# ligengen/EgoGen

Hardware: AMD Instinct MI355X
Metric: PPO env-steps/sec (512 parallel SMPL-X agents) (higher is better)
Workload: dtype f32 (blend GEMM: shape/template columns as 2-term bf16 splits, pose correctives as one fp16 product, fp32 accumulate); PPO update products on 2-term bf16 splits; rollout policy layers on 2-term bf16 splits

## Files before the change

egogen_amd/_lib.py:

```python
from __future__ import annotations

import ctypes as C
import os

_HERE = os.path.dirname(os.path.abspath(__file__))
LIB_PATH = os.path.join(_HERE, "libegogen_hip.so")

c_float_p = C.POINTER(C.c_float)
c_int_p = C.POINTER(C.c_int32)


class EgxError(RuntimeError):
    pass


class BodyModelHost(C.Structure):
    _fields_ = [
        ("num_verts", C.c_int),
        ("v_template_host", C.c_void_p), ("shapedirs_host", C.c_void_p), ("posedirs_host", C.c_void_p),
        ("J_regressor_host", C.c_void_p), ("parents_host", C.c_void_p), ("lbs_weights_host", C.c_void_p),
        ("hand_comps_l_host", C.c_void_p), ("hand_comps_r_host", C.c_void_p),
        ("hand_mean_l_host", C.c_void_p), ("hand_mean_r_host", C.c_void_p),
        ("extra_vids_host", C.c_void_p), ("lmk_vids_host", C.c_void_p), ("lmk_bary_host", C.c_void_p),
        ("num_markers", C.c_int), ("marker_vids_host", C.c_void_p),
# ... 227 lines not shown
    "egx_policy_train_create": (C.c_int, [C.POINTER(PolicyWeights), C.POINTER(PolicyGrads), C.c_int, C.POINTER(C.c_void_p)]),
    "egx_policy_train_destroy": (None, [C.c_void_p]),
    "egx_policy_train_refresh": (C.c_int, [C.c_void_p, C.c_void_p]),
    "egx_policy_train_packed": (C.c_int, [C.c_void_p, C.POINTER(PolicyPacked3)]),
    "egx_policy_train_bind": (C.c_int, [C.c_void_p, C.c_void_p, C.c_void_p]),
    "egx_policy_train_step": (C.c_int, [C.c_void_p] * 9 + [C.c_float] * 6 + [C.c_void_p, C.c_void_p]),
    "egx_policy_train_step_heads": (C.c_int, [C.c_void_p] * 9 + [C.c_float] * 6 + [C.c_void_p, C.c_void_p]),
    "egx_policy_train_step_encoders": (C.c_int, [C.c_void_p, C.c_void_p]),
    "egx_policy_train_set_precision": (C.c_int, [C.c_void_p, C.c_int]),
    "egx_policy_train_dense3_launches": (C.c_int, [C.c_void_p]),
    "egx_policy_train_head": (C.c_int, [C.c_void_p, C.POINTER(UpdateHead), C.c_void_p]),
    "egx_policy_train_step_cursor": (C.c_int, [C.c_void_p, C.POINTER(UpdateHead), C.c_void_p] + [C.c_float] * 6 + [C.c_void_p]),
    "egx_policy_train_step_heads_cursor": (C.c_int, [C.c_void_p, C.POINTER(UpdateHead), C.c_void_p] + [C.c_float] * 6 + [C.c_void_p]),
    "egx_adamw_clip_step_cursor": (C.c_int, [C.c_void_p, C.c_void_p, C.c_void_p, C.c_void_p, C.c_size_t, C.c_size_t, C.c_float] +
                                   [C.c_double] * 5 + [C.c_void_p, C.c_void_p, C.c_void_p, C.c_void_p]),
    "egx_pack3_bytes": (C.c_size_t, [C.c_int, C.c_int]),
    "egx_pack3": (C.c_int, [C.c_void_p, C.c_int, C.c_int, C.c_int, C.c_int, C.c_void_p, C.c_int, C.c_int, C.c_void_p]),
    "egx_gemm3_workspace_bytes": (C.c_size_t, [C.c_int, C.c_int, C.c_int]),
    "egx_gemm3": (C.c_int, [C.c_void_p, C.c_int, C.c_int, C.c_void_p, C.c_int, C.c_int, C.c_int, C.c_int, C.c_int, C.c_void_p, C.c_int,
                            C.c_float, C.c_void_p, C.c_int, C.c_void_p, C.c_int, C.c_void_p, C.c_int, C.c_void_p, C.c_size_t, C.c_void_p]),
    "egx_vposer_workspace_bytes": (C.c_size_t, [C.c_int]),
    "egx_vposer_encode": (C.c_int, [C.POINTER(VposerWeights), C.c_void_p, C.c_int, C.c_int, C.c_void_p, C.c_void_p,
                                    C.c_size_t, C.c_void_p]),
}

_lib = None


def load():
    global _lib
# ... 38 lines not shown
```

egogen_amd/csrc/egx_nets.h:

```cpp
#pragma once
#include "egx_common.h"
#include "egx_frame.h"

struct EgxSeg {
  const float* p;
  int w, ld;
};

int egx_launch_linear(hipStream_t st, int M, int N, const EgxSeg* segs, int nseg, const float* W, const float* b,
                      int act, float slope, const float* res, int ldr, float* out, int ldo);
int egx_launch_gru_pointwise(hipStream_t st, const float* gi, const float* gh, const float* hprev, int ldh, float* hout,
                             int ldo, int M, int H);
int egx_launch_cont6d_to_aa(hipStream_t st, const float* xb6, int n, float* out, int ldo);
int egx_launch_posenc(hipStream_t st, const float* dist, const float* time, int A, float* out);

void egx_launch_frame_scan(hipStream_t st, float* y, const float* x_last, int x_ld, int A, int width, int T);

struct D3Pack {
  const float* src;
  int R, K, ld, col0;
  void* dst;
  int S_total, s0;
  int transpose = 0;
};
// ... 26 lines not shown
  int S3T = 0, s3T0 = 0;
  float* bias_out = nullptr;
  int n_split = 0;
};
constexpr int EGX_DENSE3_MAX = 12;
int egx_launch_dense3_n(hipStream_t st, const D3Plain* ps, int n);
enum { EGX_DENSE3_BASE = 0, EGX_DENSE3_DEEP = 1, EGX_DENSE3_WIDE = 2 };
int egx_dense3_config(const D3Plain* ps, int n);
void egx_launch_dense3(hipStream_t st, const D3Plain& p);
void egx_launch_dense3_pair(hipStream_t st, const D3Plain& p, const D3Plain& q);
void egx_launch_dense3_triple(hipStream_t st, const D3Plain& p, const D3Plain& q, const D3Plain& r);
int egx_ppo_loss_packed_precleared(const float* zp, const float* value, const float* act, const float* adv, const float* ret,
                                   const float* logp_old, const float* adv_stats, const float* scale, float adv_eps, float min_logvar,
                                   float max_logvar, float eps_clip, float vf_coef, float ent_coef, int num_rows, float* g_zp,
                                   float* g_value, float* out_terms, void* stream_, const int* cursor = nullptr, int max_cursor = 0);
void egx_launch_posenc3(hipStream_t st, const float* dist, const float* time, int n, float* out, int ld, void* out3, int S3, int s0,
                        void* out3T = nullptr, int S3T = 0, int col0T = 0, float* zero6 = nullptr );

#if defined(__HIPCC__)
struct EgxRowsIdentity {
  __device__ __forceinline__ size_t operator()(int r) const { return (size_t)r; }
};
struct EgxRowsGathered {
  const long long* __restrict__ idx;
  int num_src;
  __device__ __forceinline__ size_t operator()(int r) const {
    const long long s = idx[r];
    return (size_t)min(max(s, 0LL), (long long)num_src - 1);
  }
};
// ... 97 lines not shown
```

egogen_amd/csrc/ppo.hip:

```cpp
#include <algorithm>
#include <cstring>
#include "egx_nets.h"

namespace {
constexpr float LOG_SQRT_2PI = 0.91893853320467274178f;

}

__device__ __forceinline__ float egx_wave_sum(float v) {
#pragma unroll
  for (int o = 32; o > 0; o >>= 1) v += __shfl_xor(v, o);
  return v;
}

__global__ __launch_bounds__(256) void egx_ppo_loss_kernel(const float* __restrict__ mu, const float* __restrict__ logvar,
                                                          const float* __restrict__ value, const float* __restrict__ act,
                                                          const float* __restrict__ adv, const float* __restrict__ ret,
                                                          const float* __restrict__ logp_old, const float* __restrict__ adv_stats,
                                                          const float* __restrict__ scale_ptr, float adv_eps, float min_lv,
                                                          float max_lv, float eps_clip, float vf_coef, float ent_coef, int n,
                                                          int stride ,
                                                          float* __restrict__ g_mu, float* __restrict__ g_logvar,
                                                          float* __restrict__ g_value, float* __restrict__ out_terms,
                                                          const int* __restrict__ cursor, int max_cursor) {
// ... 252 lines not shown
    const double t = (double)*step;
    const float bc1 = (float)(1.0 - pow(b1, t)), bc2 = (float)(1.0 - pow(b2, t));
    float coef = 1.f;
    if (do_clip) coef = fminf(max_norm / ((float)sqrt(red[0]) + 1e-6f), 1.f);
    consts[0] = coef;
    consts[1] = (float)(lr / bc1);
    consts[2] = sqrtf(bc2);
    if (cursor) *cursor += 1;
  }
}

__global__ __launch_bounds__(256) void egx_adamw_flat_kernel(float* __restrict__ p, const float* __restrict__ g, float* __restrict__ m,
                                                             float* __restrict__ v, size_t n, size_t n_clip,
                                                             const float* __restrict__ consts ,
                                                             double lr, double b1, double b2, double eps, double wd) {
  const float coef = consts[0], step_size = consts[1], bc2s = consts[2];
  const size_t i0 = ((size_t)blockIdx.x * 256 + threadIdx.x) * 4;
  if (i0 >= n) return;
  const int cnt = (int)((n - i0 < 4) ? (n - i0) : 4);
  float gr[4], pv[4], mv[4], vv[4];
  if (cnt == 4) {
    *reinterpret_cast<float4*>(gr) = *reinterpret_cast<const float4*>(g + i0);
    *reinterpret_cast<float4*>(pv) = *reinterpret_cast<const float4*>(p + i0);
    *reinterpret_cast<float4*>(mv) = *reinterpret_cast<const float4*>(m + i0);
    *reinterpret_cast<float4*>(vv) = *reinterpret_cast<const float4*>(v + i0);
  } else {
    for (int e = 0; e < cnt; ++e) { gr[e] = g[i0 + e]; pv[e] = p[i0 + e]; mv[e] = m[i0 + e]; vv[e] = v[i0 + e]; }
  }
  const double omb1 = 1.0 - b1, omb2 = 1.0 - b2, lrwd = lr * wd;
#pragma unroll
  for (int e = 0; e < 4; ++e) {
    if (e < cnt) {
      float gg = gr[e];
      if (i0 + e < n_clip) gg *= coef;
      pv[e] = (float)((double)pv[e] - lrwd * (double)pv[e]);
      mv[e] = (float)((double)mv[e] + omb1 * ((double)gg - (double)mv[e]));
      vv[e] = (float)(b2 * (double)vv[e] + omb2 * (double)gg * (double)gg);
      const float denom = (float)((double)(sqrtf(vv[e]) / bc2s) + eps);
      pv[e] -= step_size * mv[e] / denom;
    }
  }
  if (cnt == 4) {
    *reinterpret_cast<float4*>(p + i0) = *reinterpret_cast<const float4*>(pv);
    *reinterpret_cast<float4*>(m + i0) = *reinterpret_cast<const float4*>(mv);
    *reinterpret_cast<float4*>(v + i0) = *reinterpret_cast<const float4*>(vv);
  } else {
    for (int e = 0; e < cnt; ++e) { p[i0 + e] = pv[e]; m[i0 + e] = mv[e]; v[i0 + e] = vv[e]; }
  }
}

__global__ void egx_zero_terms_kernel(float* __restrict__ t) {
  if (threadIdx.x < 6) t[threadIdx.x] = 0.f;
}

static int ppo_loss_blocks(int num_rows) { return std::max(1, std::min(256, egx_ceil_div(num_rows, 8))); }

// ... 112 lines not shown
extern "C" int egx_rollout_store(const float* state, const float* egosensing, const float* dist, const float* time, const float* rew,
                                 const int32_t* term, int num_agents, float* state_dst, float* ego_dst, float* dist_dst, float* time_dst,
                                 float* rew_dst, int32_t* term_dst, float* ep_ret, float* ep_len, float* done_sums, void* stream_) {
  EGX_REQUIRE(state && egosensing && dist && time && state_dst && ego_dst && dist_dst && time_dst && num_agents > 0, "bad arguments");
  EGX_REQUIRE((!rew_dst && !term_dst && !ep_ret) || (rew && term && rew_dst && term_dst), "reward / termination source or slot missing");
  EGX_REQUIRE(!ep_ret || (ep_len && done_sums && rew && term), "episode bookkeeping needs ep_len, done_sums, rew, term");
  hipLaunchKernelGGL(egx_rollout_store_kernel, dim3(num_agents + (ep_ret ? 1 : 0)), dim3(256), 0, static_cast<hipStream_t>(stream_), state,
                     egosensing, dist, time, rew, term, num_agents, state_dst, ego_dst, dist_dst, time_dst, rew_dst, term_dst, ep_ret, ep_len,
                     done_sums);
  EGX_HIP_CHECK(hipGetLastError());
  return EGX_OK;
}

extern "C" size_t egx_adamw_workspace_floats(void) { return 1024 + 8; }

static int adamw_clip_step(float* param, const float* grad, float* exp_avg, float* exp_avg_sq, size_t n, size_t n_clip,
                           float max_norm, double lr, double beta1, double beta2, double eps, double weight_decay,
                           float* step, float* workspace, int* cursor, void* stream_) {
  EGX_REQUIRE(param && grad && exp_avg && exp_avg_sq && step && workspace && n > 0 && n_clip <= n, "bad arguments");
  hipStream_t st = static_cast<hipStream_t>(stream_);
  const int nb = 1024;
  const bool do_clip = max_norm > 0.f && n_clip > 0;
  hipLaunchKernelGGL(egx_sumsq_partial_kernel, dim3(nb), dim3(256), 0, st, grad, do_clip ? n_clip : (size_t)0, workspace, step);
  hipLaunchKernelGGL(egx_adamw_consts_kernel, dim3(1), dim3(256), 0, st, workspace, nb, do_clip ? 1 : 0, max_norm, lr, beta1, beta2,
                     step, workspace + nb, cursor);
  const size_t blocks = (n + 1023) / 1024;
  hipLaunchKernelGGL(egx_adamw_flat_kernel, dim3((unsigned)blocks), dim3(256), 0, st, param, grad, exp_avg, exp_avg_sq, n, n_clip,
                     workspace + nb, lr, beta1, beta2, eps, weight_decay);
  EGX_HIP_CHECK(hipGetLastError());
  return EGX_OK;
}

extern "C" int egx_adamw_clip_step(float* param, const float* grad, float* exp_avg, float* exp_avg_sq, size_t n, size_t n_clip,
                                   float max_norm, double lr, double beta1, double beta2, double eps, double weight_decay,
                                   float* step, float* workspace, void* stream_) {
  return adamw_clip_step(param, grad, exp_avg, exp_avg_sq, n, n_clip, max_norm, lr, beta1, beta2, eps, weight_decay, step, workspace,
                         nullptr, stream_);
}

extern "C" int egx_adamw_clip_step_cursor(float* param, const float* grad, float* exp_avg, float* exp_avg_sq, size_t n, size_t n_clip,
                                          float max_norm, double lr, double beta1, double beta2, double eps, double weight_decay,
                                          float* step, float* workspace, int32_t* cursor, void* stream_) {
  return adamw_clip_step(param, grad, exp_avg, exp_avg_sq, n, n_clip, max_norm, lr, beta1, beta2, eps, weight_decay, step, workspace,
                         cursor, stream_);
}
```

egogen_amd/csrc/update3.hip:

```cpp
#include <algorithm>
#include <cstdlib>
#include <cstring>
#include <vector>
#include "d3.h"

namespace {

struct PackEntry {
  const float* src;
  int red, cols, ld, col0;
  bf16x8* dst;
  int S_total, s0;
  int transpose;
  int ones_row;
  int frag_end;
  bf16x8* dst2;
  int S_total2;
};

template <class Rows>
__device__ __forceinline__ void u3_pack_fragment(const PackEntry& e, const float* __restrict__ src, int frag, int lane, int nplanes,
                                                 const Rows& rows) {
  float x[8];
  int rt, s;
// ... 67 lines not shown
    __builtin_amdgcn_wave_barrier();
#pragma unroll
    for (int t = 0; t < 2; ++t) {
#pragma unroll
      for (int q = 0; q < 8; ++q) x[q] = sb[8 * kg + q][16 * t + r];
      bf16x8 pl[3];
      d3_split(x, pl);
      bf16x8* o = e.dst2 + ((size_t)(2 * bj + t) * e.S_total2 + bi) * 3 * 64 + lane;
#pragma unroll
      for (int p = 0; p < 3; ++p)
        if (p < nplanes) o[p * 64] = pl[p];
    }
    return;
  }
  u3_pack_fragment(e, e.src, frag, lane, nplanes, EgxRowsIdentity());
}

struct HeadArgs {
  const PackEntry* tab;
  int n_tab, frags_tab, nplanes;
  const float *state, *ego;
  const long long* perm;
  const int* cursor;
  int max_cursor, n, num_src;
  const float *dist, *time, *act, *adv, *ret, *logp;
  float *act_c, *adv_c, *ret_c, *logp_c;
  float* stats;
  float* log;
  float* pe_out;
  int pe_ld;
// ... 171 lines not shown
struct egx_policy_train {
  int n = 0, Sn = 0;
  Arena ar;
  Encoder enc[2];
  Branch br[2];
  float* catf = nullptr;
  bf16x8 *cat_r = nullptr, *catT = nullptr;
  PackEntry* tab_weights = nullptr; int n_weights = 0, frags_weights = 0;
  PackEntry* tab_inputs = nullptr; int n_inputs = 0, frags_inputs = 0;
  PackEntry* tab_loss = nullptr; int n_loss = 0, frags_loss = 0;
  std::vector<PackEntry> h_inputs;
  const float* bound_state = nullptr; const float* bound_ego = nullptr;
  int prec = 0;
  int dense3_launches = 0;
  bool merge = true;
};

namespace {

int upload_table(std::vector<PackEntry>& v, PackEntry** dev, int* frags) {
  int run = 0;
  for (PackEntry& e : v) {
    if (e.transpose == 2) {
      run += egx_ceil_div(e.red, 32) * egx_ceil_div(e.cols, 32);
    } else {
      const int rows = e.transpose ? e.cols + (e.ones_row >= 0 ? 1 : 0) : e.red;
      const int red = e.transpose ? e.red : e.cols;
      run += (int)d3_img_frags(rows, red);
    }
    e.frag_end = run;
// ... 42 lines not shown
  const int lane = (row & 15) + 16 * kg;
  bf16x8 one;
#pragma unroll
  for (int e = 0; e < 8; ++e) one[e] = (short)0x3F80;
  img[((size_t)(row >> 4) * S_total + s) * 3 * 64 + lane] = one;
}

}

extern "C" int egx_policy_train_create(const egx_policy_weights* w, const egx_policy_grads* g, int num_rows, egx_policy_train** out) {
  EGX_REQUIRE(w && g && out, "null argument");
  EGX_REQUIRE(num_rows > 0 && num_rows % 32 == 0, "the minibatch must be a multiple of 32 rows");
  auto* h = new egx_policy_train();
  h->n = num_rows; h->Sn = num_rows / 32;
  if (const char* e = getenv("EGX_UPDATE_MERGE")) h->merge = !(e[0] == '0' && e[1] == 0);
  Encoder& X = h->enc[0];
  X.Wih = w->x_enc_w_ih; X.Whh = w->x_enc_w_hh; X.bih = w->x_enc_b_ih; X.bhh = w->x_enc_b_hh;
  X.gWih = g->x_enc_w_ih; X.gWhh = g->x_enc_w_hh; X.gbih = g->x_enc_b_ih; X.gbhh = g->x_enc_b_hh;
  X.in_dim = ST_DIM; X.cat_off = 0;
  Encoder& E = h->enc[1];
  E.Wih = w->ego_enc_w_ih; E.Whh = w->ego_enc_w_hh; E.bih = w->ego_enc_b_ih; E.bhh = w->ego_enc_b_hh;
  E.gWih = g->ego_enc_w_ih; E.gWhh = g->ego_enc_w_hh; E.gbih = g->ego_enc_b_ih; E.gbhh = g->ego_enc_b_hh;
  E.in_dim = EGO_DIM; E.cat_off = HD;
  for (int l = 0; l < 4; ++l) {
    h->br[0].W[l] = w->actor_w[l]; h->br[0].b[l] = w->actor_b[l]; h->br[0].gW[l] = g->actor_w[l]; h->br[0].gb[l] = g->actor_b[l];
    h->br[1].W[l] = w->critic_w[l]; h->br[1].b[l] = w->critic_b[l]; h->br[1].gW[l] = g->critic_w[l]; h->br[1].gb[l] = g->critic_b[l];
  }
  h->br[0].Wout = w->actor_out_w; h->br[0].bout = w->actor_out_b; h->br[0].gWout = g->actor_out_w; h->br[0].gbout = g->actor_out_b;
  h->br[0].nout = ZP;
  h->br[1].Wout = w->critic_out_w; h->br[1].bout = w->critic_out_b; h->br[1].gWout = g->critic_out_w; h->br[1].gbout = g->critic_out_b;
// ... 35 lines not shown
  for (int e = 0; e < 2; ++e) {
    Encoder& En = h->enc[e];
    add(tw, En.Wih, 3 * HD, En.in_dim, En.in_dim, 0, En.Wih_r, egx_ceil_div(En.in_dim, 32), 0, 0, -1);
    add_both(tw, En.Whh, 3 * HD, HD, En.Whh_r, En.Whh_t);
  }
  for (int b = 0; b < 2; ++b) {
    Branch& B = h->br[b];
    for (int l = 0; l < 4; ++l) {
      add_both(tw, B.W[l], CAT, CAT, B.W_r[l], B.W_t[l]);
    }
    add_both(tw, B.Wout, B.nout, CAT, B.Wout_r, B.Wout_t);
  }
  h->n_weights = (int)tw.size();
  int rc = upload_table(tw, &h->tab_weights, &h->frags_weights);
  if (rc) return fail(rc);
  for (int e = 0; e < 2; ++e) {
    Encoder& En = h->enc[e];
    const int d = En.in_dim, S = egx_ceil_div(d, 32);
    add(h->h_inputs, nullptr, n, d, 2 * d, 0, En.x0_r, S, 0, 0, -1);
    add(h->h_inputs, nullptr, n, d, 2 * d, d, En.x1_r, S, 0, 0, -1);
    add(h->h_inputs, nullptr, n, d, 2 * d, 0, En.xT, 2 * Sn, 0, 1, d);
    add(h->h_inputs, nullptr, n, d, 2 * d, d, En.xT, 2 * Sn, Sn, 1, d);
  }
  h->n_inputs = (int)h->h_inputs.size();
  if ((rc = upload_table(h->h_inputs, &h->tab_inputs, &h->frags_inputs))) return fail(rc);
  std::vector<PackEntry> tl;
  for (int b = 0; b < 2; ++b) {
    Branch& B = h->br[b];
    add(tl, B.ghead, n, B.nout, B.nout, 0, B.ghead_r, egx_ceil_div(B.nout, 32), 0, 0, -1);
    add(tl, B.ghead, n, B.nout, B.nout, 0, B.gheadT, Sn, 0, 1, -1);
  }
  h->n_loss = (int)tl.size();
  if ((rc = upload_table(tl, &h->tab_loss, &h->frags_loss))) return fail(rc);
  U3_CHECK(hipDeviceSynchronize());
#undef U3_CHECK
  *out = h;
  return EGX_OK;
}

extern "C" void egx_policy_train_destroy(egx_policy_train* h) {
  if (!h) return;
  (void)hipFree(h->ar.base); (void)hipFree(h->tab_weights); (void)hipFree(h->tab_inputs); (void)hipFree(h->tab_loss);
  delete h;
}

extern "C" int egx_policy_train_refresh(egx_policy_train* h, void* stream) {
  EGX_REQUIRE(h, "null handle");
  const int planes = std::max(d3_planes(h->prec), d3_planes(egx_policy_get_precision()));
  run_table(static_cast<hipStream_t>(stream), h->tab_weights, h->n_weights, h->frags_weights, planes);
  EGX_HIP_CHECK(hipGetLastError());
  return EGX_OK;
}

extern "C" int egx_policy_train_set_precision(egx_policy_train* h, int prec) {
  EGX_REQUIRE(h, "null handle");
  EGX_REQUIRE(prec == 0 || prec == 1 || prec == 2, "precision must be 0 (three bf16 planes: fp32-equivalent), 2 (two planes) or 1 (bf16)");
  h->prec = prec;
  return EGX_OK;
}

extern "C" int egx_policy_train_dense3_launches(const egx_policy_train* h) { return h ? h->dense3_launches : -1; }

extern "C" int egx_policy_train_packed(const egx_policy_train* h, egx_policy_packed3* out) {
  EGX_REQUIRE(h && out, "null argument");
  out->x_enc_w_ih = h->enc[0].Wih_r; out->x_enc_w_hh = h->enc[0].Whh_r;
  out->ego_enc_w_ih = h->enc[1].Wih_r; out->ego_enc_w_hh = h->enc[1].Whh_r;
// ... 304 lines not shown
```

egogen_amd/ppo_policy.py:

```python
from __future__ import annotations

import contextlib
import ctypes as C
import math
import os
import warnings
from typing import Dict, List, Optional

import numpy as np
import torch
import torch.distributed as dist
from torch import nn

from . import _lib
from .models import ActorCritic, GAMMAActor, GAMMACritic, GAMMAPolicyBase, PolicyHipRunner

_EPS = float(np.finfo(np.float32).eps)
_LOG_SQRT_2PI = math.log(math.sqrt(2 * math.pi))
_UPDATE_PREC = {"f32": 0, "bf16x2": 2, "bf16": 1}
_LOSS_ROWS, _OBS_ROWS = ("act", "adv", "ret", "logp_old"), ("state", "egosensing", "dist", "time")


class RunningMeanStd:

# ... 269 lines not shown
        g = _lib.PolicyGrads()
        s, a, c = self.shared_net, self.actor.pnet, self.critic.vnet
        gp = lambda t: t.grad.data_ptr()
        g.x_enc_w_ih, g.x_enc_w_hh, g.x_enc_b_ih, g.x_enc_b_hh = gp(s.x_enc.weight_ih_l0), gp(s.x_enc.weight_hh_l0), gp(s.x_enc.bias_ih_l0), gp(s.x_enc.bias_hh_l0)
        g.ego_enc_w_ih, g.ego_enc_w_hh, g.ego_enc_b_ih, g.ego_enc_b_hh = (gp(s.ego_enc.weight_ih_l0), gp(s.ego_enc.weight_hh_l0),
                                                                            gp(s.ego_enc.bias_ih_l0), gp(s.ego_enc.bias_hh_l0))
        for b in range(2):
            for k in range(2):
                g.actor_w[2 * b + k], g.actor_b[2 * b + k] = gp(a.layers[b].layers[k].weight), gp(a.layers[b].layers[k].bias)
                g.critic_w[2 * b + k], g.critic_b[2 * b + k] = gp(c.layers[b].layers[k].weight), gp(c.layers[b].layers[k].bias)
        g.actor_out_w, g.actor_out_b = gp(a.out_fc.weight), gp(a.out_fc.bias)
        g.critic_out_w, g.critic_out_b = gp(c.out_fc.weight), gp(c.out_fc.bias)
        h = C.c_void_p()
        _lib.check(lib.egx_policy_train_create(C.byref(w), C.byref(g), int(n), C.byref(h)), "egx_policy_train_create")
        _lib.check(lib.egx_policy_train_set_precision(h, _UPDATE_PREC[self.update_precision]), "egx_policy_train_set_precision")
        f = dict(dtype=torch.float32, device=self._flat_grad.device)
        head = os.environ.get("EGX_UPDATE_HEAD", "1") != "0"
        obs = [] if head else [torch.empty(n, k, **f) for k in (804, 64, 1, 1)]
        loss = [torch.empty(n, k, **f) for k in (128, 1, 1, 1)]
        if not head:
            _lib.check(lib.egx_policy_train_bind(h, _lib.ptr(obs[0]), _lib.ptr(obs[1])), "egx_policy_train_bind")
        packed = _lib.PolicyPacked3()
        _lib.check(lib.egx_policy_train_packed(h, C.byref(packed)), "egx_policy_train_packed")
        hs = {"h": h, "n": int(n), "head": head, "packed": packed, "stats": torch.zeros(2, **f),
              **dict(zip(_LOSS_ROWS, loss)), **dict(zip(_OBS_ROWS, obs))}
        self._train_handles[n] = hs
        if len(self._train_handles) == 1:
            self._runner.adopt_packed(packed, refresh=self._refresh_images)
        self._refresh_images()
        return hs

    def _chain_shapes_ok(self) -> bool:
        ok = getattr(self, "_chain_ok", None)
        if ok is None:
            a, c, s = self.actor.pnet, self.critic.vnet, self.shared_net
            def block_ok(blk, nout):
                return (blk.residual and len(blk.layers) == 2 and blk.out_fc.out_features == nout and blk.out_fc.in_features == 1152
                        and all(m.act_name == "lrelu" and len(m.layers) == 2 and
                                all(fc.in_features == 1152 and fc.out_features == 1152 for fc in m.layers) for m in blk.layers))
# ... 8 lines not shown
        self._train_handles = {}
        self._runner._wstruct = None

    def __del__(self):
        try:
            self._drop_train_handles()
        except Exception:
            pass

    def _prec_key(self):
        return (int(_lib.load().egx_policy_get_precision()), self.update_precision)

    def _img_key_now(self):
        return (sum(int(p._version) for p in self.parameters()), self._prec_key())

    def _refresh_images(self):
        if not self._train_handles:
            return
        lib, st = _lib.load(), _lib.current_stream_ptr()
        for hs in self._train_handles.values():
            _lib.check(lib.egx_policy_train_refresh(hs["h"], st), "egx_policy_train_refresh")
        self._img_key = self._img_key_now()
        self.refresh_counts["total"] += 1

    def _refresh_images_if_stale(self, who: str):
        if self._train_handles and self._img_key != self._img_key_now():
            self._refresh_images()
            self.refresh_counts[who] += 1

    def _fwd_bwd_train_step(self, hs, batch, idx, gstats, log_out, part: str = "all", cursor=None):
        if part == "encoders":
            _lib.check(_lib.load().egx_policy_train_step_encoders(hs["h"], _lib.current_stream_ptr()), "egx_policy_train_step_encoders")
        elif hs["head"]:
            self._train_step_head(hs, batch, idx, gstats, log_out, part, cursor)
        else:
            self._train_step_compact(hs, batch, idx, gstats, log_out, part)
# ... 54 lines not shown
        v_s = batch.values[:batch.n].reshape(-1).index_select(0, idx) if self._value_clip else None
        loss, terms = self.minibatch_loss(obs, act, adv, ret, lpo, gstats, v_s=v_s)
        self._flat_grad.zero_()
        loss.backward()
        if adv.is_cuda and self.use_fused_loss and self.use_fused_linear:
            from . import models as _m
            if _m._TWO_STREAM_UPDATE:
                torch.cuda.current_stream().wait_stream(_m._side_stream(adv.device))
        packed = terms.get("_packed")
        if packed is not None:
            log_out.copy_(packed)
        else:
            log_out.copy_(torch.stack([terms[k].detach() for k in ("loss", "loss/clip", "loss/vf", "loss/ent", "loss/kld", "approx_kl")]))
        return "autograd"

    def _clip_and_step(self, cursor=None):
        if self.use_flat_optimizer and self._flat_opt_state == "ready":
            g = self.optim.param_groups[0]
            lib = _lib.load()
            b1, b2 = g["betas"]
            args = (_lib.ptr(self._flat_p), _lib.ptr(self._flat_grad), _lib.ptr(self._flat_m), _lib.ptr(self._flat_v),
                    self._flat_p.numel(), self._n_clip, float(self._grad_norm or 0.0), float(g["lr"]), float(b1),
                    float(b2), float(g["eps"]), float(g["weight_decay"]), _lib.ptr(self._step_t), _lib.ptr(self._adamw_ws))
            if cursor is None:
                rc = lib.egx_adamw_clip_step(*args, _lib.current_stream_ptr())
            else:
                rc = lib.egx_adamw_clip_step_cursor(*args, _lib.ptr(cursor), _lib.current_stream_ptr())
            _lib.check(rc, "egx_adamw_clip_step")
            self._runner.mark_dirty()
            self._refresh_images()
            return
        if cursor is not None:
            raise _lib.EgxError("a minibatch cursor needs the flat optimiser")
        if self._grad_norm:
            nn.utils.clip_grad_norm_(self._actor_critic.parameters(), max_norm=self._grad_norm)
        self.optim.step()
        self._refresh_images()

    def _flat_optimizer_ready(self) -> bool:
        if self._flat_opt_state == "unsupported":
            return False
        opt = self.optim
        params = [p for g in opt.param_groups for p in g["params"]]
        if self._flat_opt_state is None:
            ok = (isinstance(opt, torch.optim.AdamW) and len(opt.param_groups) == 1 and not opt.param_groups[0].get("amsgrad", False)
# ... 146 lines not shown
            with torch.cuda.graph(g1b, pool=g1.pool()):
                fwd_bwd(part="encoders")
        if self._dp:
            g2 = torch.cuda.CUDAGraph()
            with torch.cuda.graph(g2, pool=g1.pool()):
                clip_and_step()
        return {"g1": g1, "g1b": g1b, "g2": g2, "path": path}

    def _graphs_for(self, batch: RolloutBatch, local_bs: int) -> dict:
        key = (id(batch), local_bs)
        st = self._graph_cache.get(key)
        if st is not None:
            return st
        st = self._new_graph_state(batch, local_bs)
        fwd_bwd = lambda part=None: self._graph_fwd_bwd(batch, local_bs, st, part)
        clip_and_step = lambda: self._clip_and_step(st["cursor"])
        try:
            with self._warmed_up(lambda: (fwd_bwd(), clip_and_step())):
                halves = self._dp and self.overlap_allreduce and len(self._grad_buckets()) == 2 and self._train_handle(local_bs) is not None
                st.update(self._capture(fwd_bwd, clip_and_step, halves))
            st["prec_key"] = self._prec_key()
            if st["cursor"] is not None:
                st["cursor"].zero_()
            self._refresh_images()
        except Exception as e:
            warnings.warn(f"PPO update graph capture failed ({type(e).__name__}: {e}); running the update eagerly")
            st["g1"] = st["g2"] = None
            st["failed"] = True
        self._graph_cache[key] = st
        return st

# ... 50 lines not shown
                comm.wait_stream(main)
                with torch.cuda.stream(comm):
                    self._all_reduce_grad(b1)
                main.wait_stream(comm)
            else:
                self._all_reduce_grad()
            st["g2"].replay()
        return None if st["head"] else st["log"].clone()

    def _eager_minibatch(self, batch: RolloutBatch, idx: torch.Tensor, gstats_row):
        gstats = (gstats_row[0], gstats_row[1], gstats_row[2]) if self._dp else None
        log = torch.zeros(6, device=idx.device)
        path = self._fwd_bwd(batch, idx, gstats, log)
        if self._dp:
            self._all_reduce_grad()
        self._clip_and_step()
        return log, path

    def _learn_stats(self, batch: RolloutBatch, logs: List[torch.Tensor], kld_rows: List[torch.Tensor]) -> Dict[str, List[float]]:
        names = ("loss", "loss/clip", "loss/vf", "loss/ent", "loss/kld")
        if not logs:
            return {k: [] for k in names}
        L = torch.stack(logs)[:, :5].contiguous()
        mu2 = batch.mu.reshape(batch.n * batch.A, -1).pow(2).mean(1)
        if len({int(r.shape[0]) for r in kld_rows}) == 1:
            kld = 0.5 * mu2.index_select(0, torch.cat(kld_rows)).reshape(len(kld_rows), -1).mean(1)
        else:
            kld = torch.stack([0.5 * mu2.index_select(0, r).mean() for r in kld_rows])
        L[:, 4] = kld / self.world_size if self._dp else kld
        if self._dp:
            dist.all_reduce(L)
# ... 55 lines not shown
```

include/egogen_hip.h:

```cpp
#ifndef EGOGEN_HIP_H
#define EGOGEN_HIP_H

#include <stddef.h>
#include <stdint.h>

#ifdef __cplusplus
extern "C" {
#endif

#define EGX_OK 0
#define EGX_ERR_ARG (-1)
#define EGX_ERR_HIP (-2)
#define EGX_ERR_WORKSPACE (-3)
#define EGX_ERR_CONVERGENCE (-4)

#define EGX_NUM_JOINTS 55
#define EGX_NUM_JOINTS_OUT 127
#define EGX_XB_DIM 93
#define EGX_MAX_CANDIDATES 256
#define EGX_MAX_BEAM 32
#define EGX_MAX_OBSTACLES 32
#define EGX_GEODESIC_OFF 1.0e4f
#define EGX_GEODESIC_BATCH 8
#define EGX_NUM_BETAS 10
// ... 493 lines not shown
int egx_adv_stats(const float* adv, int n, float* out_mean_std, void* stream);

int egx_track_episode(const float* rew, const int32_t* term, int num_agents, float* ep_ret, float* ep_len, float* done_sums,
                      void* stream);
int egx_rollout_store(const float* state, const float* egosensing, const float* dist, const float* time, const float* rew,
                      const int32_t* term, int num_agents, float* state_dst, float* ego_dst, float* dist_dst, float* time_dst,
                      float* rew_dst, int32_t* term_dst, float* ep_ret, float* ep_len, float* done_sums, void* stream);

size_t egx_adamw_workspace_floats(void);
int egx_adamw_clip_step(float* param, const float* grad, float* exp_avg, float* exp_avg_sq, size_t n, size_t n_clip,
                        float max_norm, double lr, double beta1, double beta2, double eps, double weight_decay, float* step,
                        float* workspace, void* stream);
int egx_adamw_clip_step_cursor(float* param, const float* grad, float* exp_avg, float* exp_avg_sq, size_t n, size_t n_clip,
                               float max_norm, double lr, double beta1, double beta2, double eps, double weight_decay, float* step,
                               float* workspace, int32_t* cursor, void* stream);

#ifdef __cplusplus
}
#endif
#endif
```

Measured before the change: 195,100.

## Fuse AdamW update with packed bf16 weight-image refresh in one kernel

Adds a table-driven kernel that applies the AdamW step to each weight fragment and writes the updated values straight into the packed bf16 split images, including the transposed copy, with leftover parameters handled by remainder blocks. This removes the separate full-parameter AdamW pass and the following refresh/pack pass that re-read the parameters. It is enabled by default through a new flat-binding call and can be turned off by environment variable. In exchange the AdamW element math is moved into a shared helper and the update kernel becomes more complex, with a shared-memory transpose and a binary search per fragment.

```diff
diff --git a/egogen_amd/_lib.py b/egogen_amd/_lib.py
--- a/egogen_amd/_lib.py
+++ b/egogen_amd/_lib.py
@@ -265,6 +265,11 @@
     "egx_policy_train_step_heads_cursor": (C.c_int, [C.c_void_p, C.POINTER(UpdateHead), C.c_void_p] + [C.c_float] * 6 + [C.c_void_p]),
     "egx_adamw_clip_step_cursor": (C.c_int, [C.c_void_p, C.c_void_p, C.c_void_p, C.c_void_p, C.c_size_t, C.c_size_t, C.c_float] +
                                    [C.c_double] * 5 + [C.c_void_p, C.c_void_p, C.c_void_p, C.c_void_p]),
+    "egx_policy_train_bind_flat": (C.c_int, [C.c_void_p, C.c_void_p, C.c_size_t]),
+    "egx_policy_train_fused_tail": (C.c_int, [C.c_void_p]),
+    "egx_adamw_clip_step_train": (C.c_int, [C.c_void_p] * 5 + [C.c_size_t, C.c_size_t, C.c_float] + [C.c_double] * 5 + [C.c_void_p] * 3),
+    "egx_adamw_clip_step_train_cursor": (C.c_int, [C.c_void_p] * 5 + [C.c_size_t, C.c_size_t, C.c_float] + [C.c_double] * 5 +
+                                         [C.c_void_p] * 4),
     "egx_pack3_bytes": (C.c_size_t, [C.c_int, C.c_int]),
     "egx_pack3": (C.c_int, [C.c_void_p, C.c_int, C.c_int, C.c_int, C.c_int, C.c_void_p, C.c_int, C.c_int, C.c_void_p]),
     "egx_gemm3_workspace_bytes": (C.c_size_t, [C.c_int, C.c_int, C.c_int]),
diff --git a/egogen_amd/csrc/adamw.h b/egogen_amd/csrc/adamw.h
--- /dev/null
+++ b/egogen_amd/csrc/adamw.h
@@ -0,0 +1,22 @@
+#pragma once
+#include "egx_common.h"
+
+struct EgxAdamwK {
+  float coef, step_size, bc2s;
+  double b2, eps, omb1, omb2, lrwd;
+  __device__ __forceinline__ EgxAdamwK(const float* __restrict__ consts, double lr, double b1, double b2_, double eps_, double wd)
+      : coef(consts[0]), step_size(consts[1]), bc2s(consts[2]), b2(b2_), eps(eps_), omb1(1.0 - b1), omb2(1.0 - b2_), lrwd(lr * wd) {}
+};
+
+static __device__ __forceinline__ void egx_adamw_elem(float& p, float g, float& m, float& v, bool clip, const EgxAdamwK& k) {
+#pragma clang fp contract(off)
+  float gg = g;
+  if (clip) gg *= k.coef;
+  const double gd = (double)gg, pd = (double)p, md = (double)m;
+  float pn = (float)__builtin_fma(-k.lrwd, pd, pd);
+  const float mn = (float)__builtin_fma(k.omb1, gd - md, md);
+  const float vn = (float)__builtin_fma(k.omb2 * gd, gd, k.b2 * (double)v);
+  const float denom = (float)((double)(sqrtf(vn) / k.bc2s) + k.eps);
+  pn -= k.step_size * mn / denom;
+  p = pn; m = mn; v = vn;
+}
diff --git a/egogen_amd/csrc/egx_nets.h b/egogen_amd/csrc/egx_nets.h
--- a/egogen_amd/csrc/egx_nets.h
+++ b/egogen_amd/csrc/egx_nets.h
@@ -64,6 +64,12 @@
                                    const float* logp_old, const float* adv_stats, const float* scale, float adv_eps, float min_logvar,
                                    float max_logvar, float eps_clip, float vf_coef, float ent_coef, int num_rows, float* g_zp,
                                    float* g_value, float* out_terms, void* stream_, const int* cursor = nullptr, int max_cursor = 0);
+constexpr int EGX_ADAMW_CONSTS = 1024;
+int egx_adamw_launch_consts(const float* grad, size_t n_clip, float max_norm, double lr, double beta1, double beta2, float* step,
+                            float* workspace, int* cursor, hipStream_t st);
+int egx_adamw_clip_step_launches(float* param, const float* grad, float* exp_avg, float* exp_avg_sq, size_t n, size_t n_clip,
+                                 float max_norm, double lr, double beta1, double beta2, double eps, double weight_decay, float* step,
+                                 float* workspace, int* cursor, void* stream_);
 void egx_launch_posenc3(hipStream_t st, const float* dist, const float* time, int n, float* out, int ld, void* out3, int S3, int s0,
                         void* out3T = nullptr, int S3T = 0, int col0T = 0, float* zero6 = nullptr );
 
diff --git a/egogen_amd/csrc/ppo.hip b/egogen_amd/csrc/ppo.hip
--- a/egogen_amd/csrc/ppo.hip
+++ b/egogen_amd/csrc/ppo.hip
@@ -1,5 +1,6 @@
 #include <algorithm>
 #include <cstring>
+#include "adamw.h"
 #include "egx_nets.h"
 
 namespace {
@@ -290,7 +291,7 @@
                                                              float* __restrict__ v, size_t n, size_t n_clip,
                                                              const float* __restrict__ consts ,
                                                              double lr, double b1, double b2, double eps, double wd) {
-  const float coef = consts[0], step_size = consts[1], bc2s = consts[2];
+  const EgxAdamwK k(consts, lr, b1, b2, eps, wd);
   const size_t i0 = ((size_t)blockIdx.x * 256 + threadIdx.x) * 4;
   if (i0 >= n) return;
   const int cnt = (int)((n - i0 < 4) ? (n - i0) : 4);
@@ -303,19 +304,9 @@
   } else {
     for (int e = 0; e < cnt; ++e) { gr[e] = g[i0 + e]; pv[e] = p[i0 + e]; mv[e] = m[i0 + e]; vv[e] = v[i0 + e]; }
   }
-  const double omb1 = 1.0 - b1, omb2 = 1.0 - b2, lrwd = lr * wd;
-#pragma unroll
-  for (int e = 0; e < 4; ++e) {
-    if (e < cnt) {
-      float gg = gr[e];
-      if (i0 + e < n_clip) gg *= coef;
-      pv[e] = (float)((double)pv[e] - lrwd * (double)pv[e]);
-      mv[e] = (float)((double)mv[e] + omb1 * ((double)gg - (double)mv[e]));
-      vv[e] = (float)(b2 * (double)vv[e] + omb2 * (double)gg * (double)gg);
-      const float denom = (float)((double)(sqrtf(vv[e]) / bc2s) + eps);
-      pv[e] -= step_size * mv[e] / denom;
-    }
-  }
+#pragma unroll
+  for (int e = 0; e < 4; ++e)
+    if (e < cnt) egx_adamw_elem(pv[e], gr[e], mv[e], vv[e], i0 + e < n_clip, k);
   if (cnt == 4) {
     *reinterpret_cast<float4*>(p + i0) = *reinterpret_cast<const float4*>(pv);
     *reinterpret_cast<float4*>(m + i0) = *reinterpret_cast<const float4*>(mv);
@@ -458,19 +449,27 @@
 
 extern "C" size_t egx_adamw_workspace_floats(void) { return 1024 + 8; }
 
-static int adamw_clip_step(float* param, const float* grad, float* exp_avg, float* exp_avg_sq, size_t n, size_t n_clip,
-                           float max_norm, double lr, double beta1, double beta2, double eps, double weight_decay,
-                           float* step, float* workspace, int* cursor, void* stream_) {
-  EGX_REQUIRE(param && grad && exp_avg && exp_avg_sq && step && workspace && n > 0 && n_clip <= n, "bad arguments");
-  hipStream_t st = static_cast<hipStream_t>(stream_);
+int egx_adamw_launch_consts(const float* grad, size_t n_clip, float max_norm, double lr, double beta1, double beta2, float* step,
+                            float* workspace, int* cursor, hipStream_t st) {
   const int nb = 1024;
   const bool do_clip = max_norm > 0.f && n_clip > 0;
   hipLaunchKernelGGL(egx_sumsq_partial_kernel, dim3(nb), dim3(256), 0, st, grad, do_clip ? n_clip : (size_t)0, workspace, step);
   hipLaunchKernelGGL(egx_adamw_consts_kernel, dim3(1), dim3(256), 0, st, workspace, nb, do_clip ? 1 : 0, max_norm, lr, beta1, beta2,
                      step, workspace + nb, cursor);
+  EGX_HIP_CHECK(hipGetLastError());
+  return EGX_OK;
+}
+
+int egx_adamw_clip_step_launches(float* param, const float* grad, float* exp_avg, float* exp_avg_sq, size_t n, size_t n_clip,
+                                 float max_norm, double lr, double beta1, double beta2, double eps, double weight_decay,
+                                 float* step, float* workspace, int* cursor, void* stream_) {
+  EGX_REQUIRE(param && grad && exp_avg && exp_avg_sq && step && workspace && n > 0 && n_clip <= n, "bad arguments");
+  hipStream_t st = static_cast<hipStream_t>(stream_);
+  const int rc = egx_adamw_launch_consts(grad, n_clip, max_norm, lr, beta1, beta2, step, workspace, cursor, st);
+  if (rc) return rc;
   const size_t blocks = (n + 1023) / 1024;
   hipLaunchKernelGGL(egx_adamw_flat_kernel, dim3((unsigned)blocks), dim3(256), 0, st, param, grad, exp_avg, exp_avg_sq, n, n_clip,
-                     workspace + nb, lr, beta1, beta2, eps, weight_decay);
+                     workspace + EGX_ADAMW_CONSTS, lr, beta1, beta2, eps, weight_decay);
   EGX_HIP_CHECK(hipGetLastError());
   return EGX_OK;
 }
@@ -478,13 +477,13 @@
 extern "C" int egx_adamw_clip_step(float* param, const float* grad, float* exp_avg, float* exp_avg_sq, size_t n, size_t n_clip,
                                    float max_norm, double lr, double beta1, double beta2, double eps, double weight_decay,
                                    float* step, float* workspace, void* stream_) {
-  return adamw_clip_step(param, grad, exp_avg, exp_avg_sq, n, n_clip, max_norm, lr, beta1, beta2, eps, weight_decay, step, workspace,
-                         nullptr, stream_);
+  return egx_adamw_clip_step_launches(param, grad, exp_avg, exp_avg_sq, n, n_clip, max_norm, lr, beta1, beta2, eps, weight_decay, step,
+                                      workspace, nullptr, stream_);
 }
 
 extern "C" int egx_adamw_clip_step_cursor(float* param, const float* grad, float* exp_avg, float* exp_avg_sq, size_t n, size_t n_clip,
                                           float max_norm, double lr, double beta1, double beta2, double eps, double weight_decay,
                                           float* step, float* workspace, int32_t* cursor, void* stream_) {
-  return adamw_clip_step(param, grad, exp_avg, exp_avg_sq, n, n_clip, max_norm, lr, beta1, beta2, eps, weight_decay, step, workspace,
-                         cursor, stream_);
-}
+  return egx_adamw_clip_step_launches(param, grad, exp_avg, exp_avg_sq, n, n_clip, max_norm, lr, beta1, beta2, eps, weight_decay, step,
+                                      workspace, cursor, stream_);
+}
diff --git a/egogen_amd/csrc/update3.hip b/egogen_amd/csrc/update3.hip
--- a/egogen_amd/csrc/update3.hip
+++ b/egogen_amd/csrc/update3.hip
@@ -1,7 +1,10 @@
 #include <algorithm>
 #include <cstdlib>
 #include <cstring>
+#include <string>
+#include <utility>
 #include <vector>
+#include "adamw.h"
 #include "d3.h"
 
 namespace {
@@ -105,6 +108,168 @@
     return;
   }
   u3_pack_fragment(e, e.src, frag, lane, nplanes, EgxRowsIdentity());
+}
+
+struct RemBlock { size_t start, end; };
+struct AdamwTabArgs {
+  const PackEntry* tab;
+  int n_tab, frags_tab, nplanes;
+  float* p; const float* g; float* m; float* v;
+  size_t n_clip;
+  const float* consts;
+  double lr, b1, b2, eps, wd;
+  const RemBlock* rem;
+  int b_tab, n_rem;
+};
+
+__device__ __forceinline__ bool u3_aligned16(const void* a, const void* b, const void* c, const void* d) {
+  return ((reinterpret_cast<uintptr_t>(a) | reinterpret_cast<uintptr_t>(b) | reinterpret_cast<uintptr_t>(c) | reinterpret_cast<uintptr_t>(d)) & 15) == 0;
+}
+__device__ __forceinline__ void u3_load8(const float* s, float (&x)[8]) {
+  const f32x4 x0 = __builtin_nontemporal_load(reinterpret_cast<const f32x4*>(s));
+  const f32x4 x1 = __builtin_nontemporal_load(reinterpret_cast<const f32x4*>(s + 4));
+  x[0] = x0[0]; x[1] = x0[1]; x[2] = x0[2]; x[3] = x0[3]; x[4] = x1[0]; x[5] = x1[1]; x[6] = x1[2]; x[7] = x1[3];
+}
+__device__ __forceinline__ void u3_store8(float* d, const float (&x)[8]) {
+  __builtin_nontemporal_store(f32x4{x[0], x[1], x[2], x[3]}, reinterpret_cast<f32x4*>(d));
+  __builtin_nontemporal_store(f32x4{x[4], x[5], x[6], x[7]}, reinterpret_cast<f32x4*>(d + 4));
+}
+struct U3Adamw8 {
+  size_t fi;
+  int valid;
+  bool fast;
+  float x[8], gr[8], mv[8], vv[8];
+};
+__device__ __forceinline__ void u3_adamw8_load(const AdamwTabArgs& a, size_t fi, int valid, U3Adamw8& w) {
+  const float *pp = a.p + fi, *gp = a.g + fi, *mp = a.m + fi, *vp = a.v + fi;
+  w.fi = fi; w.valid = valid;
+  w.fast = valid == 8 && u3_aligned16(pp, gp, mp, vp);
+  if (w.fast) {
+    u3_load8(pp, w.x); u3_load8(gp, w.gr); u3_load8(mp, w.mv); u3_load8(vp, w.vv);
+  } else {
+#pragma unroll
+    for (int q = 0; q < 8; ++q) {
+      const bool in = q < valid;
+      w.x[q] = in ? pp[q] : 0.f; w.gr[q] = in ? gp[q] : 0.f; w.mv[q] = in ? mp[q] : 0.f; w.vv[q] = in ? vp[q] : 0.f;
+    }
+  }
+}
+__device__ __forceinline__ void u3_adamw8_step(const AdamwTabArgs& a, const EgxAdamwK& k, U3Adamw8& w) {
+#pragma unroll
+  for (int q = 0; q < 8; ++q)
+    if (q < w.valid) egx_adamw_elem(w.x[q], w.gr[q], w.mv[q], w.vv[q], w.fi + q < a.n_clip, k);
+  float *pp = a.p + w.fi, *mp = a.m + w.fi, *vp = a.v + w.fi;
+  if (w.fast) {
+    u3_store8(pp, w.x); u3_store8(mp, w.mv); u3_store8(vp, w.vv);
+  } else {
+#pragma unroll
+    for (int q = 0; q < 8; ++q)
+      if (q < w.valid) { pp[q] = w.x[q]; mp[q] = w.mv[q]; vp[q] = w.vv[q]; }
+  }
+}
+
+__global__ __launch_bounds__(256) void egx_adamw_table_kernel(AdamwTabArgs a) {
+  const EgxAdamwK k(a.consts, a.lr, a.b1, a.b2, a.eps, a.wd);
+  if ((int)blockIdx.x >= a.b_tab) {
+    const int rb = (int)blockIdx.x - a.b_tab;
+    if (rb >= a.n_rem) return;
+    const RemBlock blk = a.rem[rb];
+    const size_t i0 = blk.start + 4 * (size_t)threadIdx.x;
+    if (i0 >= blk.end) return;
+    const int cnt = (int)((blk.end - i0 < 4) ? (blk.end - i0) : 4);
+    float gr[4], pv[4], mv[4], vv[4];
+    const bool vec = cnt == 4 && u3_aligned16(a.p + i0, a.g + i0, a.m + i0, a.v + i0);
+    if (vec) {
+      *reinterpret_cast<f32x4*>(gr) = *reinterpret_cast<const f32x4*>(a.g + i0);
+      *reinterpret_cast<f32x4*>(pv) = *reinterpret_cast<const f32x4*>(a.p + i0);
+      *reinterpret_cast<f32x4*>(mv) = *reinterpret_cast<const f32x4*>(a.m + i0);
+      *reinterpret_cast<f32x4*>(vv) = *reinterpret_cast<const f32x4*>(a.v + i0);
+    } else {
+#pragma unroll
+      for (int e = 0; e < 4; ++e) {
+        const bool in = e < cnt;
+        gr[e] = in ? a.g[i0 + e] : 0.f; pv[e] = in ? a.p[i0 + e] : 0.f; mv[e] = in ? a.m[i0 + e] : 0.f; vv[e] = in ? a.v[i0 + e] : 0.f;
+      }
+    }
+#pragma unroll
+    for (int e = 0; e < 4; ++e)
+      if (e < cnt) egx_adamw_elem(pv[e], gr[e], mv[e], vv[e], i0 + e < a.n_clip, k);
+    if (vec) {
+      *reinterpret_cast<f32x4*>(a.p + i0) = *reinterpret_cast<const f32x4*>(pv);
+      *reinterpret_cast<f32x4*>(a.m + i0) = *reinterpret_cast<const f32x4*>(mv);
+      *reinterpret_cast<f32x4*>(a.v + i0) = *reinterpret_cast<const f32x4*>(vv);
+    } else {
+#pragma unroll
+      for (int e = 0; e < 4; ++e)
+        if (e < cnt) { a.p[i0 + e] = pv[e]; a.m[i0 + e] = mv[e]; a.v[i0 + e] = vv[e]; }
+    }
+    return;
+  }
+  const PackEntry* __restrict__ tab = a.tab;
+  int frag = blockIdx.x * 4 + (threadIdx.x >> 6);
+  const int lane = threadIdx.x & 63, nplanes = a.nplanes;
+  if (frag >= a.frags_tab) return;
+  int lo = 0, hi = a.n_tab - 1;
+  while (lo < hi) {
+    const int mid = (lo + hi) >> 1;
+    if (frag >= tab[mid].frag_end) lo = mid + 1; else hi = mid;
+  }
+  const PackEntry e = tab[lo];
+  frag -= lo > 0 ? tab[lo - 1].frag_end : 0;
+  const size_t base = (size_t)(e.src - a.p) + e.col0;
+  float x[8];
+  if (e.transpose == 2) {
+    __shared__ float sblk[4][32][33];
+    float (*sb)[33] = sblk[threadIdx.x >> 6];
+    const int BJ = (e.cols + 31) >> 5;
+    const int bi = frag / BJ, bj = frag % BJ;
+    const int r = lane & 15, kg = lane >> 4;
+    U3Adamw8 w[2];
+#pragma unroll
+    for (int t = 0; t < 2; ++t) {
+      const int row = 32 * bi + 16 * t + r, k0 = 32 * bj + 8 * kg;
+      const int valid = row < e.red ? min(max(e.cols - k0, 0), 8) : 0;
+      u3_adamw8_load(a, valid ? base + (size_t)row * e.ld + k0 : 0, valid, w[t]);
+    }
+#pragma unroll
+    for (int t = 0; t < 2; ++t) {
+      u3_adamw8_step(a, k, w[t]);
+#pragma unroll
+      for (int q = 0; q < 8; ++q) sb[16 * t + r][8 * kg + q] = w[t].x[q];
+      bf16x8 pl[3];
+      d3_split(w[t].x, pl);
+      bf16x8* o = e.dst + ((size_t)(2 * bi + t) * e.S_total + e.s0 + bj) * 3 * 64 + lane;
+#pragma unroll
+      for (int p = 0; p < 3; ++p)
+        if (p < nplanes) o[p * 64] = pl[p];
+    }
+    __builtin_amdgcn_wave_barrier();
+#pragma unroll
+    for (int t = 0; t < 2; ++t) {
+#pragma unroll
+      for (int q = 0; q < 8; ++q) x[q] = sb[8 * kg + q][16 * t + r];
+      bf16x8 pl[3];
+      d3_split(x, pl);
+      bf16x8* o = e.dst2 + ((size_t)(2 * bj + t) * e.S_total2 + bi) * 3 * 64 + lane;
+#pragma unroll
+      for (int p = 0; p < 3; ++p)
+        if (p < nplanes) o[p * 64] = pl[p];
+    }
+    return;
+  }
+  const int S = (e.cols + 31) >> 5;
+  const int rt = frag / S, s = frag % S;
+  const int row = rt * 16 + (lane & 15), k0 = s * 32 + 8 * (lane >> 4);
+  const int valid = row < e.red ? min(max(e.cols - k0, 0), 8) : 0;
+  U3Adamw8 w;
+  u3_adamw8_load(a, valid ? base + (size_t)row * e.ld + k0 : 0, valid, w);
+  u3_adamw8_step(a, k, w);
+  bf16x8 pl[3];
+  d3_split(w.x, pl);
+  bf16x8* o = e.dst + ((size_t)rt * e.S_total + e.s0 + s) * 3 * 64 + lane;
+#pragma unroll
+  for (int p = 0; p < 3; ++p)
+    if (p < nplanes) o[p * 64] = pl[p];
 }
 
 struct HeadArgs {
@@ -306,6 +471,10 @@
   int prec = 0;
   int dense3_launches = 0;
   bool merge = true;
+  bool fused_wanted = true, fused = false;
+  std::vector<PackEntry> h_weights;
+  const float* flat_p = nullptr; size_t flat_n = 0;
+  RemBlock* rem = nullptr; int n_rem = 0;
 };
 
 namespace {
@@ -378,6 +547,7 @@
   auto* h = new egx_policy_train();
   h->n = num_rows; h->Sn = num_rows / 32;
   if (const char* e = getenv("EGX_UPDATE_MERGE")) h->merge = !(e[0] == '0' && e[1] == 0);
+  if (const char* e = getenv("EGX_UPDATE_FUSED_TAIL")) h->fused_wanted = !(e[0] == '0' && e[1] == 0);
   Encoder& X = h->enc[0];
   X.Wih = w->x_enc_w_ih; X.Whh = w->x_enc_w_hh; X.bih = w->x_enc_b_ih; X.bhh = w->x_enc_b_hh;
   X.gWih = g->x_enc_w_ih; X.gWhh = g->x_enc_w_hh; X.gbih = g->x_enc_b_ih; X.gbhh = g->x_enc_b_hh;
@@ -443,6 +613,7 @@
   h->n_weights = (int)tw.size();
   int rc = upload_table(tw, &h->tab_weights, &h->frags_weights);
   if (rc) return fail(rc);
+  h->h_weights = tw;
   for (int e = 0; e < 2; ++e) {
     Encoder& En = h->enc[e];
     const int d = En.in_dim, S = egx_ceil_div(d, 32);
@@ -470,8 +641,50 @@
 extern "C" void egx_policy_train_destroy(egx_policy_train* h) {
   if (!h) return;
   (void)hipFree(h->ar.base); (void)hipFree(h->tab_weights); (void)hipFree(h->tab_inputs); (void)hipFree(h->tab_loss);
+  (void)hipFree(h->rem);
   delete h;
 }
+
+extern "C" int egx_policy_train_bind_flat(egx_policy_train* h, const float* param, size_t n) {
+  EGX_REQUIRE(h && param && n > 0, "bad arguments");
+  h->fused = false; h->flat_p = param; h->flat_n = n;
+  auto off_tail = [&](const std::string& why) {
+    egx_set_error("egx_policy_train_bind_flat: the optimiser step keeps its two-launch tail - " + why);
+    return EGX_OK;
+  };
+  if (!h->fused_wanted) return EGX_OK;
+  std::vector<std::pair<size_t, size_t>> own;
+  const uintptr_t p0 = reinterpret_cast<uintptr_t>(param);
+  for (size_t i = 0; i < h->h_weights.size(); ++i) {
+    const PackEntry& e = h->h_weights[i];
+    const std::string which = "weight table entry " + std::to_string(i);
+    if (e.transpose != 0 && e.transpose != 2) return off_tail(which + " is a transposed view");
+    if (e.col0 != 0 || e.ld != e.cols || e.red <= 0 || e.cols <= 0) return off_tail(which + " is not a whole contiguous matrix");
+    const uintptr_t s = reinterpret_cast<uintptr_t>(e.src);
+    const size_t cnt = (size_t)e.red * e.cols;
+    if (s < p0 || (s - p0) % sizeof(float) != 0 || (s - p0) / sizeof(float) > n || cnt > n - (s - p0) / sizeof(float))
+      return off_tail(which + " does not lie wholly inside the flat parameter buffer");
+    own.emplace_back((s - p0) / sizeof(float), (s - p0) / sizeof(float) + cnt);
+  }
+  std::sort(own.begin(), own.end());
+  for (size_t i = 1; i < own.size(); ++i)
+    if (own[i].first < own[i - 1].second) return off_tail("two weight table entries overlap");
+  std::vector<RemBlock> rem;
+  size_t at = 0;
+  auto span = [&](size_t lo, size_t hi) {
+    for (; lo < hi; lo += 1024) rem.push_back({lo, std::min(lo + 1024, hi)});
+  };
+  for (const auto& o : own) { span(at, o.first); at = o.second; }
+  span(at, n);
+  (void)hipFree(h->rem);
+  h->rem = nullptr; h->n_rem = (int)rem.size();
+  EGX_HIP_CHECK(hipMalloc(reinterpret_cast<void**>(&h->rem), std::max<size_t>(1, rem.size()) * sizeof(RemBlock)));
+  if (!rem.empty()) EGX_HIP_CHECK(hipMemcpy(h->rem, rem.data(), rem.size() * sizeof(RemBlock), hipMemcpyHostToDevice));
+  h->fused = true;
+  return EGX_OK;
+}
+
+extern "C" int egx_policy_train_fused_tail(const egx_policy_train* h) { return h ? (h->fused ? 1 : 0) : -1; }
 
 extern "C" int egx_policy_train_refresh(egx_policy_train* h, void* stream) {
   EGX_REQUIRE(h, "null handle");
@@ -479,6 +692,41 @@
   run_table(static_cast<hipStream_t>(stream), h->tab_weights, h->n_weights, h->frags_weights, planes);
   EGX_HIP_CHECK(hipGetLastError());
   return EGX_OK;
+}
+
+static int adamw_clip_step_train(egx_policy_train* h, float* param, const float* grad, float* exp_avg, float* exp_avg_sq, size_t n,
+                                 size_t n_clip, float max_norm, double lr, double beta1, double beta2, double eps, double weight_decay,
+                                 float* step, float* workspace, int* cursor, void* stream_) {
+  EGX_REQUIRE(h && param && grad && exp_avg && exp_avg_sq && step && workspace && n > 0 && n_clip <= n, "bad arguments");
+  if (!(h->fused && param == h->flat_p && n == h->flat_n && h->frags_weights > 0)) {
+    const int rc = egx_adamw_clip_step_launches(param, grad, exp_avg, exp_avg_sq, n, n_clip, max_norm, lr, beta1, beta2, eps, weight_decay,
+                                                step, workspace, cursor, stream_);
+    return rc ? rc : egx_policy_train_refresh(h, stream_);
+  }
+  hipStream_t st = static_cast<hipStream_t>(stream_);
+  const int rc = egx_adamw_launch_consts(grad, n_clip, max_norm, lr, beta1, beta2, step, workspace, cursor, st);
+  if (rc) return rc;
+  AdamwTabArgs a;
+  a.tab = h->tab_weights; a.n_tab = h->n_weights; a.frags_tab = h->frags_weights;
+  a.nplanes = std::max(d3_planes(h->prec), d3_planes(egx_policy_get_precision()));
+  a.p = param; a.g = grad; a.m = exp_avg; a.v = exp_avg_sq; a.n_clip = n_clip; a.consts = workspace + EGX_ADAMW_CONSTS;
+  a.lr = lr; a.b1 = beta1; a.b2 = beta2; a.eps = eps; a.wd = weight_decay;
+  a.rem = h->rem; a.b_tab = egx_ceil_div(h->frags_weights, 4); a.n_rem = h->n_rem;
+  hipLaunchKernelGGL(egx_adamw_table_kernel, dim3(a.b_tab + a.n_rem), dim3(256), 0, st, a);
+  EGX_HIP_CHECK(hipGetLastError());
+  return EGX_OK;
+}
+extern "C" int egx_adamw_clip_step_train(egx_policy_train* h, float* param, const float* grad, float* exp_avg, float* exp_avg_sq, size_t n,
+                                         size_t n_clip, float max_norm, double lr, double beta1, double beta2, double eps,
+                                         double weight_decay, float* step, float* workspace, void* stream) {
+  return adamw_clip_step_train(h, param, grad, exp_avg, exp_avg_sq, n, n_clip, max_norm, lr, beta1, beta2, eps, weight_decay, step,
+                               workspace, nullptr, stream);
+}
+extern "C" int egx_adamw_clip_step_train_cursor(egx_policy_train* h, float* param, const float* grad, float* exp_avg, float* exp_avg_sq,
+                                                size_t n, size_t n_clip, float max_norm, double lr, double beta1, double beta2, double eps,
+                                                double weight_decay, float* step, float* workspace, int32_t* cursor, void* stream) {
+  return adamw_clip_step_train(h, param, grad, exp_avg, exp_avg_sq, n, n_clip, max_norm, lr, beta1, beta2, eps, weight_decay, step,
+                               workspace, cursor, stream);
 }
 
 extern "C" int egx_policy_train_set_precision(egx_policy_train* h, int prec) {
diff --git a/egogen_amd/ppo_policy.py b/egogen_amd/ppo_policy.py
--- a/egogen_amd/ppo_policy.py
+++ b/egogen_amd/ppo_policy.py
@@ -307,6 +307,8 @@
         h = C.c_void_p()
         _lib.check(lib.egx_policy_train_create(C.byref(w), C.byref(g), int(n), C.byref(h)), "egx_policy_train_create")
         _lib.check(lib.egx_policy_train_set_precision(h, _UPDATE_PREC[self.update_precision]), "egx_policy_train_set_precision")
+        _lib.check(lib.egx_policy_train_bind_flat(h, _lib.ptr(self._flat_p), self._flat_p.numel()), "egx_policy_train_bind_flat")
+        fused_tail = lib.egx_policy_train_fused_tail(h) == 1
         f = dict(dtype=torch.float32, device=self._flat_grad.device)
         head = os.environ.get("EGX_UPDATE_HEAD", "1") != "0"
         obs = [] if head else [torch.empty(n, k, **f) for k in (804, 64, 1, 1)]
@@ -315,7 +317,7 @@
             _lib.check(lib.egx_policy_train_bind(h, _lib.ptr(obs[0]), _lib.ptr(obs[1])), "egx_policy_train_bind")
         packed = _lib.PolicyPacked3()
         _lib.check(lib.egx_policy_train_packed(h, C.byref(packed)), "egx_policy_train_packed")
-        hs = {"h": h, "n": int(n), "head": head, "packed": packed, "stats": torch.zeros(2, **f),
+        hs = {"h": h, "n": int(n), "head": head, "fused_tail": fused_tail, "packed": packed, "stats": torch.zeros(2, **f),
               **dict(zip(_LOSS_ROWS, loss)), **dict(zip(_OBS_ROWS, obs))}
         self._train_handles[n] = hs
         if len(self._train_handles) == 1:
@@ -354,12 +356,13 @@
     def _img_key_now(self):
         return (sum(int(p._version) for p in self.parameters()), self._prec_key())
 
-    def _refresh_images(self):
+    def _refresh_images(self, fresh=None):
         if not self._train_handles:
             return
         lib, st = _lib.load(), _lib.current_stream_ptr()
         for hs in self._train_handles.values():
-            _lib.check(lib.egx_policy_train_refresh(hs["h"], st), "egx_policy_train_refresh")
+            if hs is not fresh:
+                _lib.check(lib.egx_policy_train_refresh(hs["h"], st), "egx_policy_train_refresh")
         self._img_key = self._img_key_now()
         self.refresh_counts["total"] += 1
 
@@ -444,7 +447,7 @@
             log_out.copy_(torch.stack([terms[k].detach() for k in ("loss", "loss/clip", "loss/vf", "loss/ent", "loss/kld", "approx_kl")]))
         return "autograd"
 
-    def _clip_and_step(self, cursor=None):
+    def _clip_and_step(self, cursor=None, n=None):
         if self.use_flat_optimizer and self._flat_opt_state == "ready":
             g = self.optim.param_groups[0]
             lib = _lib.load()
@@ -452,13 +455,16 @@
             args = (_lib.ptr(self._flat_p), _lib.ptr(self._flat_grad), _lib.ptr(self._flat_m), _lib.ptr(self._flat_v),
                     self._flat_p.numel(), self._n_clip, float(self._grad_norm or 0.0), float(g["lr"]), float(b1),
                     float(b2), float(g["eps"]), float(g["weight_decay"]), _lib.ptr(self._step_t), _lib.ptr(self._adamw_ws))
-            if cursor is None:
-                rc = lib.egx_adamw_clip_step(*args, _lib.current_stream_ptr())
-            else:
-                rc = lib.egx_adamw_clip_step_cursor(*args, _lib.ptr(cursor), _lib.current_stream_ptr())
-            _lib.check(rc, "egx_adamw_clip_step")
+            hs = self._train_handles.get(int(n)) if n is not None else None
+            if hs is not None and not hs["fused_tail"]:
+                hs = None
+            if hs is not None:
+                args = (hs["h"],) + args
+            tail = (_lib.current_stream_ptr(),) if cursor is None else (_lib.ptr(cursor), _lib.current_stream_ptr())
+            name = "egx_adamw_clip_step" + ("_train" if hs is not None else "") + ("" if cursor is None else "_cursor")
+            _lib.check(getattr(lib, name)(*args, *tail), name)
             self._runner.mark_dirty()
-            self._refresh_images()
+            self._refresh_images(fresh=hs)
             return
         if cursor is not None:
             raise _lib.EgxError("a minibatch cursor needs the flat optimiser")
@@ -635,7 +641,7 @@
             return st
         st = self._new_graph_state(batch, local_bs)
         fwd_bwd = lambda part=None: self._graph_fwd_bwd(batch, local_bs, st, part)
-        clip_and_step = lambda: self._clip_and_step(st["cursor"])
+        clip_and_step = lambda: self._clip_and_step(st["cursor"], n=local_bs)
         try:
             with self._warmed_up(lambda: (fwd_bwd(), clip_and_step())):
                 halves = self._dp and self.overlap_allreduce and len(self._grad_buckets()) == 2 and self._train_handle(local_bs) is not None
@@ -716,7 +722,7 @@
         path = self._fwd_bwd(batch, idx, gstats, log)
         if self._dp:
             self._all_reduce_grad()
-        self._clip_and_step()
+        self._clip_and_step(n=int(idx.shape[0]))
         return log, path
 
     def _learn_stats(self, batch: RolloutBatch, logs: List[torch.Tensor], kld_rows: List[torch.Tensor]) -> Dict[str, List[float]]:
diff --git a/include/egogen_hip.h b/include/egogen_hip.h
--- a/include/egogen_hip.h
+++ b/include/egogen_hip.h
@@ -531,6 +531,14 @@
 int egx_adamw_clip_step_cursor(float* param, const float* grad, float* exp_avg, float* exp_avg_sq, size_t n, size_t n_clip,
                                float max_norm, double lr, double beta1, double beta2, double eps, double weight_decay, float* step,
                                float* workspace, int32_t* cursor, void* stream);
+int egx_policy_train_bind_flat(egx_policy_train* h, const float* param, size_t n);
+int egx_policy_train_fused_tail(const egx_policy_train* h);
+int egx_adamw_clip_step_train(egx_policy_train* h, float* param, const float* grad, float* exp_avg, float* exp_avg_sq, size_t n,
+                              size_t n_clip, float max_norm, double lr, double beta1, double beta2, double eps, double weight_decay,
+                              float* step, float* workspace, void* stream);
+int egx_adamw_clip_step_train_cursor(egx_policy_train* h, float* param, const float* grad, float* exp_avg, float* exp_avg_sq, size_t n,
+                                     size_t n_clip, float max_norm, double lr, double beta1, double beta2, double eps,
+                                     double weight_decay, float* step, float* workspace, int32_t* cursor, void* stream);
 
 #ifdef __cplusplus
 }
```

Result: faster. 200,900, median of 6 (+3.0%).
